# Amelie-Schreiber/ShapeMol

Hardware: AMD Instinct MI355X
Metric: molecules/sec (1000-step DDPM sample, batch 256) (higher is better)
Workload: dtype f32 (matrix operands split exactly into 3 x bf16 pieces = 24 bits, six piece products, fp32 accumulate); 1 GPU; BASELINE configs[1]: batch 256 MOSES-prior molecules (9-27 atoms) per GPU, 1000-step chain, fp32 results, k=8, synthetic shapes + hash-filled weights; besides the 5 warm-up steps an untimed 200-step chain runs first to reach the loaded clocks; batch_per_gpu=256, atoms_per_gpu=5541, total_atoms=5541, noise=device Philox, trajectories=kept in HBM, launch=hipGraph replay, parallelism=dp1 (whole batches per rank), ranks_seen=1

## Files before the change

shapemol_amd/csrc/shapemol_hip.hip:

```cpp
#include "../../include/shapemol_hip.h"
#include "sm_device.h"
#include "sm_edge.h"
#include "sm_edge_bf16.h"
#include "sm_edge16.h"
#include "sm_node.h"
#include "sm_node16.h"
#include "sm_edge_stream.h"
#include "sm_misc.h"
#include "sm_cfg.h"
#include "sm_guide_groups.h"
#include "sm_mesh.h"
#include <hip/hip_ext.h>

#include <algorithm>
#include <cmath>
#include <cstdio>
#include <cstring>
#include <map>
#include <string>
#include <type_traits>
#include <vector>

#include "sm_pack.h"
#include "sm_devmem.h"
// ... 349 lines not shown
int launch_mlp2(shapemol_ctx *c, hipStream_t s, const char *name, const DevMlpImg &m, const float *in0, const float *in1,
                int mode, const float *resid, float *out, int ld_out, int n_store, int n_atoms) {
    NodeMlpArgs a{};
    a.in0 = in0; a.in1 = in1; a.w1img = c->P(m.w1img); a.b1 = c->P(m.b1); a.ln_g = c->P(m.g); a.ln_b = c->P(m.be);
    a.w2img = c->P(m.w2img); a.b2 = c->P(m.b2); a.resid = resid; a.out = out; a.ld_out = ld_out; a.n_store = n_store;
    a.mode = mode; a.nt2 = m.nt2; a.n_atoms = n_atoms;
    const int n_ct = (n_atoms + 15) / 16, teams = NodeMlpLds<H>::TEAMS;
    LAUNCH(name, SMK((node_mlp2_kernel<H, KT>), dim3((n_ct + teams - 1) / teams), dim3(kNodeThreads), 0, s, a));
    return 0;
}

template <int H>
int launch_linear(shapemol_ctx *c, hipStream_t s, const char *name, const float *in, const float *wimg, const float *wimg6, const float *wimg16, const float *add_mol,
                  int ld_add, float *out, int ld_out, int n_out_tiles, int n_atoms, unsigned long long *stamps) {
    const lg::LinGeom g = lg::linear_geom(launch_in<H>(c, n_atoms), n_out_tiles);
    const dim3 grid(g.ogroups * g.agroups), block(g.waves * 64);
    const bool f16 = c->opt.lin_bf16 && c->opt.node_f16;
    NodeLinArgs a{in, f16 ? wimg16 : (c->opt.lin_bf16 ? wimg6 : wimg), add_mol, c->mol_of, out, n_atoms, n_out_tiles, g.tpg, ld_add, ld_out, stamps, g.waves};
    if (f16) {
        const size_t shm = (size_t)std::min(g.tpg, kLin16Chunk) * 2 * H * 32;
        if (c->opt.feat_f16) LAUNCH(name, SMK((node_linear16_kernel<H, true>), grid, block, shm, s, a, c->status + ST_RANGE));
        else LAUNCH(name, SMK(node_linear16_kernel<H>, grid, block, shm, s, a, c->status + ST_RANGE));
    } else if (c->opt.lin_bf16) {
        const size_t shm = (size_t)std::min(g.tpg, kLin6Chunk) * 3 * H * 32;
        LAUNCH(name, SMK(node_linear6_kernel<H>, grid, block, shm, s, a));
    } else {
        LAUNCH(name, SMK(node_linear_kernel<H>, grid, block, 0, s, a));
    }
    return 0;
}

template <int H>
int launch_node_levels(shapemol_ctx *c, hipStream_t s, const NodeChainArgs &na, const float *lin_img6, const float *add_mol, int ld_add,
                       float *out, int ld_out, int lin_tiles, bool out_done) {
    const int n = na.n_atoms;
    const lg::NodeLevelsGeom g = lg::node_levels_geom(launch_in<H>(c, n), na.n_follow, lin_tiles);
    if (!out_done) LAUNCH("node_chain", SMK(node_out6_kernel<H>, dim3(g.n_pairs), dim3(H * 4), Out6Lds<H>::BYTES, s, na));
    NodeAfterArgs a{};
    a.f[0] = na.f[0]; a.f[1] = na.f[1];
    a.n_pairs = g.n_pairs; a.n_fjobs = g.n_fjobs; a.n_ljobs = g.n_ljobs; a.order = c->opt.after_order; a.lin_chunk = g.lin_chunk;
    a.lin = NodeLinArgs{na.h_out, lin_img6, add_mol, c->mol_of, out, n, lin_tiles, g.tpg, ld_add, ld_out, nullptr, g.lw};
    const size_t shm = After6Lds<H>::bytes(a.lin_chunk);
    const int64_t rec[8] = {1, a.n_fjobs, a.n_ljobs, g.bw, a.order, g.tpg, a.lin_chunk, (int64_t)shm};
    std::copy(rec, rec + 8, c->node_rec);
    LAUNCH("node_pre", SMK(node_after6_kernel<H>, dim3(a.n_fjobs + a.n_ljobs), dim3(g.bw * 64), shm, s, a));
    return 0;
}

NodeFollow follow_of(const shapemol_ctx *c, const DevMlpImg &m, int mode, float *out, int ld_out, int n_store) {
    NodeFollow f{};
    f.w1img = c->P(m.w1img); f.b1 = c->P(m.b1); f.ln_g = c->P(m.g); f.ln_b = c->P(m.be);
    f.w1img6 = c->P(c->opt.node_f16 ? m.w1img16 : m.w1img6); f.w2img6 = c->P(c->opt.node_f16 ? m.w2img16 : m.w2img6);
    f.w2img = c->P(m.w2img); f.b2 = c->P(m.b2); f.out = out; f.ld_out = ld_out; f.n_store = n_store; f.mode = mode; f.nt2 = m.nt2;
    return f;
}

__global__ void knn_pin_kernel(const int *off, int n_steps, const int *atom, const int *pnbr, int k, int kp, const int *step_cur, int n_atoms, int *nbr) {
    const int step = *step_cur;
    if (step < 0 || step >= n_steps) return;
    const int lo = off[step], hi = off[step + 1];
    for (int e = lo + blockIdx.x * blockDim.x + threadIdx.x; e < hi; e += gridDim.x * blockDim.x) {
        const int i = atom[e];
        if (i < 0 || i >= n_atoms) continue;
        for (int sl = 0; sl < kp; ++sl) nbr[(size_t)i * kp + sl] = sl < k ? pnbr[(size_t)e * k + sl] : -1;
    }
}

template <int H>
int run_prep_shape(shapemol_ctx *c, hipStream_t s, int64_t B, const float *d_shape, const ShapePrep &sp);

int cfg_group_blocks(int64_t n, int n_groups) { return (int)(n / 2048 + n_groups); }

CfgArgs cfg_args(const shapemol_ctx *c, int64_t N) {
    CfgArgs a{};
// ... 230 lines not shown
                sa.vf = pending;
                if (sf.out_fused) sa.no = NodeOutArgs{c->att, cur_h, c->P(Dl.no.b1), c->P(Dl.no.g), c->P(Dl.no.be), c->P(Dl.no.b2),
                                                   c->P(Dl.no.w1img6), c->P(Dl.no.w2img6), h_dst};
                if (launch_stream<H, false>(c, s, sa)) return 1;
            }
            pending = VnFold{};
            if (sf.half_tiles && launch_combine32<false>(c, s, c->att, n)) return 1;
        } else if (sf.phases && c->opt.edge_bf16 == 1) {
            EdgeFusedArgs fa{c->P(Dl.img_kx), c->P(Dl.img_vx), pre_x, c->q_x, cur_x, c->nbr, c->ew, c->alpha, c->att, n, ld_pre_x, stamps_x};
            if (launch_fused<H, false>(c, s, fa)) return 1;
        } else {
            EdgeArgs e{c->P(Dl.blob_x2h), pre_x, c->q_x, cur_x, c->nbr, c->ew, c->att, n, ld_pre_x, stamps_x};
            if (launch_edge<H, false>(c, s, e)) return 1;
        }
        {
            float *dst = h_dst;
            NodeChainArgs na{};
            na.att = c->att; na.h = cur_h; na.h_out = dst; na.n_atoms = n;
            na.stamps = (c->kstamp_sel == 3 && l == 0) ? c->kstamps : nullptr;
            na.w1img = c->P(Dl.no.w1img); na.b1 = c->P(Dl.no.b1); na.ln_g = c->P(Dl.no.g); na.ln_b = c->P(Dl.no.be);
            na.w2img = c->P(Dl.no.w2img); na.b2 = c->P(Dl.no.b2);
            na.w1img6 = c->P(c->opt.node_f16 ? Dl.no.w1img16 : Dl.no.w1img6); na.w2img6 = c->P(c->opt.node_f16 ? Dl.no.w2img16 : Dl.no.w2img6);
            na.f[0] = follow_of(c, Dl.q_h2x, NODE_LN_RELU, c->q_h, H, H);
            na.n_follow = 1;
            if (has_next) { na.f[1] = follow_of(c, c->dm.layer[l + 1].q_x2h, NODE_LN_RELU, c->q_x, H, H); na.n_follow = 2; }
            else if (out_v) { na.f[1] = follow_of(c, c->dm.vhead, NODE_SSP, out_v, C, C); na.n_follow = 2; v_done = true; }
            const int n_ct = (n + 15) / 16;
            const int lin_tiles = (has_next && l + 1 < L ? 8 : 4) * NT;
            if (sf.lin_fused) {
                na.lin_img16 = c->P(Dl.lin16_img); na.add_mol = sp.addp + (size_t)l * c->capB * 8 * H; na.mol_of = c->mol_of;
                na.pre_out = c->preAB; na.n_lin_tiles = lin_tiles; na.ld_add = 8 * H; na.ld_out = 8 * H;
            }
            float *lin_add = sp.addp + (size_t)l * c->capB * 8 * H;
            if (sf.levels) { if (launch_node_levels<H>(c, s, na, c->P(Dl.lin6_img), lin_add, 8 * H, c->preAB, 8 * H, lin_tiles, sf.out_fused)) return 1; }
            else if (sf.xc_fused) { rec[4] = 1; if (launch_x2h_chain<H>(c, s, xea, na)) return 1; }
            else if (c->opt.chain_bf16 && c->opt.node_f16 && c->opt.feat_f16) LAUNCH("node_chain", SMK((node_chain16_kernel<H, true>), dim3((n_ct + CHAIN_COLS - 1) / CHAIN_COLS), dim3(H * 4), Chain16Lds<H>::BYTES, s, na, c->status + ST_RANGE));
            else if (c->opt.chain_bf16 && c->opt.node_f16) LAUNCH("node_chain", SMK(node_chain16_kernel<H>, dim3((n_ct + CHAIN_COLS - 1) / CHAIN_COLS), dim3(H * 4), Chain16Lds<H>::BYTES, s, na, c->status + ST_RANGE));
            else if (c->opt.chain_bf16) LAUNCH("node_chain", SMK(node_chain6_kernel<H>, dim3((n_ct + CHAIN_COLS - 1) / CHAIN_COLS), dim3(H * 4), Chain6Lds<H>::BYTES, s, na));
            else LAUNCH("node_chain", SMK(node_chain_kernel<H>, dim3((n_ct + CHAIN_COLS - 1) / CHAIN_COLS), dim3(H * 4), 0, s, na));
            cur_h = dst;
            if (!sf.lin_fused && !sf.levels && launch_linear<H>(c, s, "node_pre", cur_h, c->P(Dl.lin_img), c->P(Dl.lin6_img), c->P(Dl.lin16_img), lin_add, 8 * H,
                                 c->preAB, 8 * H, lin_tiles, n, (c->kstamp_sel == 0 && l == 0) ? c->kstamps : nullptr)) return 1;
        }
        float *x_next = (last && out_pos) ? out_pos : ((cur_x == c->x_a) ? c->x_b : c->x_a);
        bool vn_done = false, stats_done = false;
        unsigned long long *stamps_h = (c->kstamp_sel == 2 && l == 0) ? c->kstamps : nullptr;
        if ((sf.f16 || sf.stream) && c->opt.vn_fuse != 1) {
            const H2xPlan plan = h2x_plan(c, sp, l, sf.fold, has_next, sf.half_tiles, stat_acc, cur_x, x_next, out_pos);
            pending = plan.pending; stats_done = plan.stats_done; vn_done = plan.vn_done;
            if (plan.ddpm.enable) c->ddpm_vf = plan.ddpm;
            rec[2] |= plan.pending.enable; rec[3] |= plan.ddpm.enable;
            if (sf.f16) {
                Edge16Args ea{};
                ea.image_k = c->P(Dl.i16_kh); ea.image_v = c->P(Dl.i16_vh);
                fill_edge(ea, c, c->preAB, 8 * H, c->q_h, cur_x, c->o3, n, sf.half_tiles, stamps_h);
                ea.vn = plan.vn; ea.xsum = plan.xsum;
                if (launch_edge16<H, true>(c, s, ea)) return 1;
            } else {
                EdgeStreamArgs sa{};
                sa.part_k = c->P(Dl.st_kh); sa.part_v = c->P(Dl.st_vh);
                sa.w2k = reinterpret_cast<const unsigned *>(c->P(Dl.sw2_kh));
                fill_edge(sa, c, c->preAB, 8 * H, c->q_h, cur_x, c->o3, n, sf.half_tiles, stamps_h);
                sa.vn = plan.vn; sa.xsum = plan.xsum;
                if (launch_stream<H, true>(c, s, sa)) return 1;
            }
            if (sf.half_tiles && launch_combine32<true>(c, s, c->o3, n)) return 1;
        } else if (sf.phases) {
// ... 290 lines not shown
    if (k == "first_step") {
        if (value < 0 || value >= c->cfg.num_timesteps) return fail("first_step must be in [0, num_timesteps)");
        c->first_step = (int)value;
        return 0;
    }
    if (k == "stop_layer") c->opt.stop_layer = (int)value;
    else if (k == "edge_bf16") {
        if (value < 0 || value > 3) return fail("edge_bf16 must be 0 (fp32 MFMA), 1 (exactly split bf16, phase kernels), 2 (exactly split bf16, streaming kernels) or 3 (two-piece f16)");
        if (value != 3 && value != 2 && c->KP > 16) return fail("k > 16 runs on the streaming (edge_bf16 = 2) or the two-piece f16 (edge_bf16 = 3) edge kernels");
        if (value == 3 && c->hid_max > 6.0e4f) return fail("edge_bf16 = 3: the edge MLPs' LayerNorm outputs may exceed the fp16 range for these weights");
        c->opt.edge_bf16 = (int)value;
    }
    else if (k == "edge_tiles") { if (value < -1 || value > 1) return fail("edge_tiles must be -1 (automatic), 0 (sliced one-job launches) or 1 (looping launch)"); c->opt.edge_tiles = (int)value; }
    else if (k == "node_f16") c->opt.node_f16 = value != 0;
    else if (k == "feat_f16") {
        if (value && (c->opt.edge_bf16 != 3 || !c->opt.node_f16)) return fail("feat_f16 = 1 needs the f16 kernels (edge_bf16 = 3, node_f16 = 1)");
        c->opt.feat_f16 = value != 0;
    }
    else if (k == "lin_fuse") c->opt.lin_fuse = value != 0;
    else if (k == "stream_whole_rounds") c->opt.stream_whole_rounds = value != 0;
    else if (k == "x2h_chain") c->opt.x2h_chain = value != 0;
    else if (k == "graph_fuse") c->opt.graph_fuse = value != 0;
    else if (k == "bn_eval") c->bn_eval = value != 0;
    else if (k == "ddpm_fold") c->opt.ddpm_fold = value != 0;
    else if (k == "vn_fold") c->opt.vn_fold = value != 0;
    else if (k == "prologue_tab") c->opt.prologue_tab = value != 0;
    else if (k == "lin_bf16") c->opt.lin_bf16 = (int)value;
    else if (k == "chain_bf16") c->opt.chain_bf16 = (int)value;
    else if (k == "vn_fuse") c->opt.vn_fuse = (int)value;
    else if (k == "node_levels") c->opt.node_levels = value != 0;
    else if (k == "x2h_out_fuse") { if (value < 0 || value > 2) return fail("x2h_out_fuse must be 0 (node_out6_kernel), 1 (x2h tail inside its boundary) or 2 (x2h tail always)"); c->opt.x2h_out_fuse = (int)value; }
    else if (k == "stream_chunk") { if (value < 0 || value > 4096) return fail("stream_chunk must be 0 (automatic) .. 4096"); c->opt.stream_chunk_opt = (int)value; }
    else if (k == "after_order") { if (value < 0 || value > 2) return fail("after_order must be 0 (follow-up jobs first), 1 (interleaved) or 2 (linear jobs first)"); c->opt.after_order = (int)value; }
    else if (k == "after_waves") { if (value < 1 || value > 16) return fail("after_waves must be 1..16"); c->opt.after_waves = (int)value; }
    else if (k == "after_lin_wgs") { if (value < 0 || value > 4096) return fail("after_lin_wgs must be 0 (automatic) .. 4096"); c->opt.after_lin_wgs = (int)value; }
    else if (k == "lin_waves") { if (value < 1 || value > 16) return fail("lin_waves must be 1..16"); c->opt.lin_waves = (int)value; }
    else if (k == "stamps") c->stamp_on = (int)value;
    else if (k == "kstamp_sel") c->kstamp_sel = (int)value;
    else if (k == "edge_waves") { if (value < 0 || value > 12) return fail("edge_waves must be 0 (automatic) .. 12"); c->opt.edge_threads = (int)value * 64; }
    else return fail("unknown option " + k);
    hipSetDevice(c->device);
    c->drop_graphs();
    return 0;
}

int64_t shapemol_debug_read(shapemol_ctx *c, const char *name, void *dst, size_t max_bytes) {
    if (!c || !name || !dst) { fail("shapemol_debug_read: null argument"); return -1; }
    const std::string k(name);
    const shapemol_config &g = c->cfg;
    const int64_t N = c->lastN;
    const void *src = nullptr; size_t bytes = 0;
    int64_t dims[8] = {N, c->lastB, c->KP, g.hidden_dim, g.n_heads, g.num_layers, c->capN, c->capB};
    if (k == "dims") { if (max_bytes < sizeof(dims)) return -1; std::memcpy(dst, dims, sizeof(dims)); return sizeof(dims); }
    if (k == "captures") { if (max_bytes < 8) return -1; std::memcpy(dst, &c->n_captures, 8); return 8; }
    if (k == "launch") { if (max_bytes < sizeof(c->launch_rec)) return -1; std::memcpy(dst, c->launch_rec, sizeof(c->launch_rec)); return sizeof(c->launch_rec); }
    if (k == "launch_x2h_out") { if (max_bytes < sizeof(c->x2h_out_rec)) return -1; std::memcpy(dst, c->x2h_out_rec, sizeof(c->x2h_out_rec)); return sizeof(c->x2h_out_rec); }
    if (k == "launch_node") { if (max_bytes < sizeof(c->node_rec)) return -1; std::memcpy(dst, c->node_rec, sizeof(c->node_rec)); return sizeof(c->node_rec); }
    if (k == "nbr") { src = c->nbr; bytes = N * c->KP * 4; }
    else if (k == "ew") { src = c->ew; bytes = N * c->KP * 4; }
    else if (k == "h") { src = c->last_h; bytes = N * g.hidden_dim * 4; }
    else if (k == "x") { src = c->last_x; bytes = N * 3 * 4; }
    else if (k == "h0") { src = c->h_a; bytes = N * g.hidden_dim * 4; }
    else if (k == "q_x") { src = c->q_x; bytes = N * g.hidden_dim * 4; }
    else if (k == "pre0") { src = c->pre0; bytes = N * 4 * g.hidden_dim * 4; }
    else if (k == "add0") { src = c->prep[0].add0; bytes = (size_t)c->lastB * 4 * g.hidden_dim * 4; }
    else if (k == "pre") { src = c->preAB; bytes = N * 8 * g.hidden_dim * 4; }
// ... 176 lines not shown
```

shapemol_amd/csrc/sm_device.h:

```cpp
#pragma once
#include <hip/hip_runtime.h>
#include <stdint.h>

typedef float f32x4 __attribute__((ext_vector_type(4)));

#define SM_DEV __device__ __forceinline__

#ifdef SM_STAMPS
#define SM_STAMP(buf, slot)                                                                        \
    do {                                                                                           \
        if ((buf) != nullptr && (threadIdx.x & 63) == 0) {                                         \
            unsigned long long t_;                                                                 \
            __builtin_amdgcn_sched_barrier(0);                                                     \
            asm volatile("s_waitcnt vmcnt(0) lgkmcnt(0)\n\ts_memrealtime %0\n\ts_waitcnt lgkmcnt(0)" : "=s"(t_)::"memory"); \
            __builtin_amdgcn_sched_barrier(0);                                                     \
            (buf)[(((size_t)blockIdx.y * gridDim.x + blockIdx.x) * (blockDim.x >> 6) + (threadIdx.x >> 6)) * 8 + (slot)] = t_; \
        }                                                                                          \
    } while (0)
#define SM_TICK(buf, slot)                                                                         \
    do {                                                                                           \
        if ((buf) != nullptr && (threadIdx.x & 63) == 0) {                                         \
            unsigned long long t_;                                                                 \
            __builtin_amdgcn_sched_barrier(0);                                                     \
            asm volatile("s_memrealtime %0\n\ts_waitcnt lgkmcnt(0)" : "=s"(t_)::"memory");         \
            __builtin_amdgcn_sched_barrier(0);                                                     \
            (buf)[(((size_t)blockIdx.y * gridDim.x + blockIdx.x) * (blockDim.x >> 6) + (threadIdx.x >> 6)) * 8 + (slot)] = t_; \
        }                                                                                          \
    } while (0)
#else
#define SM_STAMP(buf, slot) do { } while (0)
#define SM_TICK(buf, slot) do { } while (0)
#endif

SM_DEV f32x4 mfma16(float a, float b, f32x4 c) {
    return __builtin_amdgcn_mfma_f32_16x16x4f32(a, b, c, 0, 0, 0);
}

SM_DEV float4 ldg4(const float *p) { return *reinterpret_cast<const float4 *>(p); }
SM_DEV void stg4(float *p, float4 v) { *reinterpret_cast<float4 *>(p) = v; }

SM_DEV void copy_to_lds(float *lds, const float *g, int n4, int tid, int nthr) {
    const float4 *src = reinterpret_cast<const float4 *>(g);
    float4 *dst = reinterpret_cast<float4 *>(lds);
    constexpr int U = 8;
    int i = tid;
    for (; i + (U - 1) * nthr < n4; i += U * nthr) {
        float4 v[U];
#pragma unroll
        for (int u = 0; u < U; ++u) v[u] = src[i + u * nthr];
#pragma unroll
        for (int u = 0; u < U; ++u) dst[i + u * nthr] = v[u];
    }
    for (; i < n4; i += nthr) dst[i] = src[i];
}

SM_DEV void dma_to_lds(float *lds, const float *g, int n4, int wave, int nwave, int lane) {
    typedef __attribute__((address_space(3))) void lds_void;
    typedef __attribute__((address_space(1))) const void gbl_void;
    const int wu = __builtin_amdgcn_readfirstlane(wave);
    for (int c = wu; c < n4 / 64; c += nwave)
        __builtin_amdgcn_global_load_lds((gbl_void *)(g + ((size_t)c * 64 + lane) * 4), (lds_void *)(lds + (size_t)c * 256), 16, 0, 0);
}

SM_DEV void image_to_lds(float *lds, const float *g, int n4, int tid, int wave, int nwave, int lane) {
// ... 254 lines not shown
```

shapemol_amd/csrc/sm_launch.h:

```cpp
#pragma once
#include <algorithm>

namespace lg {

struct Options {
    int stop_layer = -1, edge_threads = 0 , lin_waves = 16, edge_bf16 = 2, lin_bf16 = 1, chain_bf16 = 1, vn_fuse = 2;
    int vn_fold = 1;
    int max_mol_atoms = 0;
    int stream_whole_rounds = 0;
    int lin_fuse = 0;
    int ddpm_fold = 1;
    int graph_fuse = 1;
    int x2h_chain = 1;
    int node_levels = 1;
    int x2h_out_fuse = 1;
    int stream_chunk_opt = 0;
    int after_order = 2;
    int after_waves = 16;
    int after_lin_wgs = 0;
    int node_f16 = 0;
    int feat_f16 = 0;
    int edge_tiles = -1;
    int prologue_tab = 1;
};

struct KernelConsts { int vn_fold_cap, stream_tpr, chain_cols, graph_cap, lin6_chunk; bool chain16_fits; };

struct In { Options o; KernelConsts k; int KP, num_cu, H, n_atoms; };

inline int cdiv(int a, int b) { return (a + b - 1) / b; }

struct Jobs { int apj, jobs; bool half; };
inline Jobs tile_jobs(int KP, int n_atoms) {
    const int apj = KP >= 16 ? 1 : 16 / KP;
    return {apj, KP > 16 ? 2 * n_atoms : cdiv(n_atoms, apj), KP > 16};
}

enum class Form { One, Loop, Sliced, Strided };
struct EdgeGeom { Form form; int apj, jobs, waves, grid, chunk, slice, atoms_per_wg; };

inline int edge_waves(const In &in, int jobs) {
    return in.o.edge_threads > 0 ? in.o.edge_threads / 64 : std::max(4, std::min(12, cdiv(jobs, in.num_cu)));
}
inline EdgeGeom one_job_geom(const In &in, int waves) {
    const Jobs j = tile_jobs(in.KP, in.n_atoms);
    const int grid = std::max(1, std::min(in.num_cu, cdiv(j.jobs, waves)));
    return {j.jobs <= grid * waves ? Form::One : Form::Strided, j.apj, j.jobs, waves, grid, waves, grid * waves, j.half ? 0 : waves * j.apj};
}

inline EdgeGeom edge_fp32_geom(const In &in) {
    const Jobs j = tile_jobs(in.KP, in.n_atoms);
    const int grid = std::max(1, std::min(in.num_cu, j.jobs));
    return {Form::Strided, j.apj, j.jobs, in.o.edge_threads > 0 ? in.o.edge_threads / 64 : 12, grid, 1, grid, 0};
}

inline EdgeGeom edge_phase_geom(const In &in) {
// ... 110 lines not shown
```

shapemol_amd/csrc/sm_node.h:

```cpp
#pragma once
#include "sm_device.h"

enum NodeMode { NODE_LN_RELU = 1, NODE_SSP = 2 };
constexpr int kNodeThreads = 1024;

struct NodeLinArgs {
    const float *in;
    const float *wimg;
    const float *add_mol;
    const int *mol_of;
    float *out;
    int n_atoms, n_out_tiles, tiles_per_group;
    int ld_add, ld_out;
    unsigned long long *stamps;
    int nwave;
};

constexpr int kLinChunk = 8;

template <int H>
__global__ void __launch_bounds__(kNodeThreads)
node_linear_kernel(NodeLinArgs a) {
    constexpr int NT = H / 16;
    constexpr int XS = H + 16;
    __shared__ __attribute__((aligned(16))) float tiles[kLinChunk * 16 * XS];
    const int lane = threadIdx.x & 63, wave = threadIdx.x >> 6;
    const int n = lane & 15, g = lane >> 4;
    const int nwave = blockDim.x >> 6;
    const int ogroups = (a.n_out_tiles + nwave - 1) / nwave;
    const int ot_raw = (blockIdx.x % ogroups) * nwave + wave;
    const bool ot_ok = ot_raw < a.n_out_tiles;
    const int ot = ot_ok ? ot_raw : a.n_out_tiles - 1;
    const int ag = blockIdx.x / ogroups;
    const int n_ct = (a.n_atoms + 15) / 16;
// ... 8 lines not shown
        const int nc = min(kLinChunk, ct1 - cb);
        __syncthreads();
        for (int idx = threadIdx.x; idx < nc * 16 * (H / 4); idx += blockDim.x) {
            const int ar = idx / (H / 4), c4 = idx % (H / 4);
            const int at = min(cb * 16 + ar, a.n_atoms - 1);
            stg4(tiles + ar * XS + 4 * c4, ldg4(a.in + (size_t)at * H + 4 * c4));
        }
        __syncthreads();
        float4 add_cur = {0.f, 0.f, 0.f, 0.f}, add_nxt = {0.f, 0.f, 0.f, 0.f};
        if (a.add_mol) add_cur = ldg4(a.add_mol + (size_t)a.mol_of[min(cb * 16 + n, a.n_atoms - 1)] * a.ld_add + 16 * ot + 4 * g);
        for (int c = 0; c < nc; ++c) {
            if (a.add_mol && c + 1 < nc)
                add_nxt = ldg4(a.add_mol + (size_t)a.mol_of[min((cb + c + 1) * 16 + n, a.n_atoms - 1)] * a.ld_add + 16 * ot + 4 * g);
            const float *xrow = tiles + (c * 16 + n) * XS;
            f32x4 acc = {add_cur.x, add_cur.y, add_cur.z, add_cur.w};
#pragma unroll
            for (int t = 0; t < NT; ++t) {
                const float4 x = ldg4(xrow + 16 * t + 4 * g);
                acc = mfma16(w[t].x, x.x, acc);
                acc = mfma16(w[t].y, x.y, acc);
                acc = mfma16(w[t].z, x.z, acc);
                acc = mfma16(w[t].w, x.w, acc);
            }
            const int atom = (cb + c) * 16 + n;
            if (ot_ok && atom < a.n_atoms) stg4(a.out + (size_t)atom * a.ld_out + 16 * ot + 4 * g, float4{acc[0], acc[1], acc[2], acc[3]});
            add_cur = add_nxt;
        }
    }
    SM_STAMP(a.stamps, 2);
}

constexpr int kLin6Chunk = 8;

template <int H>
SM_DEV void linear6_job(const NodeLinArgs &a, int job, int chunk, u32x4 *frag) {
    constexpr int NB = H / 32;
    const int lane = threadIdx.x & 63, wave = threadIdx.x >> 6;
    const int n = lane & 15, g = lane >> 4;
    const int nwave = a.nwave;
    const int ogroups = (a.n_out_tiles + nwave - 1) / nwave;
    const int ot_raw = (job % ogroups) * nwave + wave;
    const bool ot_ok = ot_raw < a.n_out_tiles;
    const int ot = ot_ok ? ot_raw : a.n_out_tiles - 1;
    const int ag = job / ogroups;
    const int n_ct = (a.n_atoms + 15) / 16;
    const int ct0 = ag * a.tiles_per_group, ct1 = min(ct0 + a.tiles_per_group, n_ct);

    u32x4 w[3][NB];
    {
        const u32x4 *wi = reinterpret_cast<const u32x4 *>(a.wimg) + (size_t)ot * 3 * NB * 64 + lane;
#pragma unroll
        for (int p = 0; p < 3; ++p)
#pragma unroll
            for (int b = 0; b < NB; ++b) w[p][b] = wi[(p * NB + b) * 64];
    }

    for (int cb = ct0; cb < ct1; cb += chunk) {
        const int nc = min(chunk, ct1 - cb);
        __syncthreads();
        for (int idx = threadIdx.x; idx < nc * NB * 64; idx += nwave * 64) {
            const int sl = idx & 63, sb = (idx >> 6) % NB, sc = idx / (64 * NB);
            const int at = min((cb + sc) * 16 + (sl & 15), a.n_atoms - 1);
            const float *src = a.in + (size_t)at * H + 32 * sb + 4 * (sl >> 4);
            const float4 v0 = ldg4(src), v1 = ldg4(src + 16);
            const float v[8] = {v0.x, v0.y, v0.z, v0.w, v1.x, v1.y, v1.z, v1.w};
            u32x4 hi, mid, lo;
            split3_bf16(v, hi, mid, lo);
            u32x4 *dst = frag + ((size_t)(sc * 3) * NB + sb) * 64 + sl;
            dst[0] = hi; dst[NB * 64] = mid; dst[2 * NB * 64] = lo;
        }
        __syncthreads();
        for (int c = 0; c < nc; c += 2) {
            const bool two = c + 1 < nc;
            const int atom0 = (cb + c) * 16 + n, atom1 = atom0 + 16;
            f32x4 acc0 = {0.f, 0.f, 0.f, 0.f}, acc1 = {0.f, 0.f, 0.f, 0.f};
            if (a.add_mol) {
                const float4 t0 = ldg4(a.add_mol + (size_t)a.mol_of[min(atom0, a.n_atoms - 1)] * a.ld_add + 16 * ot + 4 * g);
                const float4 t1 = ldg4(a.add_mol + (size_t)a.mol_of[min(atom1, a.n_atoms - 1)] * a.ld_add + 16 * ot + 4 * g);
                acc0 = f32x4{t0.x, t0.y, t0.z, t0.w}; acc1 = f32x4{t1.x, t1.y, t1.z, t1.w};
            }
            const u32x4 *f0 = frag + (size_t)(c * 3) * NB * 64 + lane;
            const u32x4 *f1 = frag + (size_t)((two ? c + 1 : c) * 3) * NB * 64 + lane;
#pragma unroll
            for (int b = 0; b < NB; ++b) {
                const u32x4 h0 = f0[b * 64], m0 = f0[(NB + b) * 64], l0 = f0[(2 * NB + b) * 64];
                const u32x4 h1 = f1[b * 64], m1 = f1[(NB + b) * 64], l1 = f1[(2 * NB + b) * 64];
                acc0 = mfma_bf16(w[2][b], h0, acc0); acc1 = mfma_bf16(w[2][b], h1, acc1);
                acc0 = mfma_bf16(w[1][b], m0, acc0); acc1 = mfma_bf16(w[1][b], m1, acc1);
                acc0 = mfma_bf16(w[0][b], l0, acc0); acc1 = mfma_bf16(w[0][b], l1, acc1);
                acc0 = mfma_bf16(w[1][b], h0, acc0); acc1 = mfma_bf16(w[1][b], h1, acc1);
                acc0 = mfma_bf16(w[0][b], m0, acc0); acc1 = mfma_bf16(w[0][b], m1, acc1);
                acc0 = mfma_bf16(w[0][b], h0, acc0); acc1 = mfma_bf16(w[0][b], h1, acc1);
            }
            if (ot_ok && atom0 < a.n_atoms) stg4(a.out + (size_t)atom0 * a.ld_out + 16 * ot + 4 * g, float4{acc0[0], acc0[1], acc0[2], acc0[3]});
            if (ot_ok && two && atom1 < a.n_atoms) stg4(a.out + (size_t)atom1 * a.ld_out + 16 * ot + 4 * g, float4{acc1[0], acc1[1], acc1[2], acc1[3]});
        }
    }
}

template <int H>
__global__ void __launch_bounds__(kNodeThreads)
node_linear6_kernel(NodeLinArgs a) {
    extern __shared__ __attribute__((aligned(16))) unsigned char lin6_lds[];
    linear6_job<H>(a, blockIdx.x, kLin6Chunk, reinterpret_cast<u32x4 *>(lin6_lds));
}

struct NodeMlpArgs {
    const float *in0;
    const float *in1;
    const float *w1img;
    const float *b1;
    const float *ln_g, *ln_b;
    const float *w2img;
    const float *b2;
    const float *resid;
    float *out;
    int ld_out, n_store, mode, nt2, n_atoms;
};

template <int H>
struct NodeMlpLds {
    static constexpr int NT = H / 16;
    static constexpr int TEAMS = (16 / NT) < 4 ? (16 / NT) : 4;
    static constexpr int XS = H + 16;
    static constexpr int TOTAL = TEAMS * 16 * XS;
};

template <int H, int KT>
__global__ void __launch_bounds__(kNodeThreads)
node_mlp2_kernel(NodeMlpArgs a) {
// ... 712 lines not shown
    SM_DEV void put_frag(u32x4 *fo, int sb, int sc, int sl, const float (&v)[8]) const {
        u32x4 hi, mid, lo;
        split3_bf16(v, hi, mid, lo);
        u32x4 *dst = fo + (sb * CC + sc) * 64 + frag_slot(sb, sl);
        dst[0] = hi; dst[KB * CC * 64] = mid; dst[2 * KB * CC * 64] = lo;
    }
    SM_DEV void normalise(const float *pre, int mode, const float *gam, const float *bet, u32x4 *fo) const {
        const int col = ot * (64 / LPC) + lane / LPC, ln = lane % LPC;
        const int b = ln >> 2, gg = ln & 3;
        const int fa = 32 * b + 4 * gg;
        const float4 p0 = ldg4(pre + col * XS + fa), p1 = ldg4(pre + col * XS + fa + 16);
        float v[8] = {p0.x, p0.y, p0.z, p0.w, p1.x, p1.y, p1.z, p1.w};
        if (mode == NODE_LN_RELU) {
            float s = 0.f;
#pragma unroll
            for (int i = 0; i < 8; ++i) s += v[i];
            const float mean = seg_sum<LPC>(s) * (1.0f / H);
            float q = 0.f;
#pragma unroll
            for (int i = 0; i < 8; ++i) { const float d = v[i] - mean; q += d * d; }
            const float var = seg_sum<LPC>(q) * (1.0f / H);
            const float rstd = 1.0f / sqrtf(var + 1e-5f);
            const float4 g0 = ldg4(gam + fa), g1 = ldg4(gam + fa + 16), b0 = ldg4(bet + fa), b1 = ldg4(bet + fa + 16);
            const float ga[8] = {g0.x, g0.y, g0.z, g0.w, g1.x, g1.y, g1.z, g1.w};
            const float be[8] = {b0.x, b0.y, b0.z, b0.w, b1.x, b1.y, b1.z, b1.w};
#pragma unroll
            for (int i = 0; i < 8; ++i) v[i] = fmaxf((v[i] - mean) * rstd * ga[i] + be[i], 0.f);
        } else {
#pragma unroll
            for (int i = 0; i < 8; ++i) v[i] = (v[i] > 20.f ? v[i] : log1pf(expf(v[i]))) - 0.6931471805599453f;
        }
        put_frag<NB>(fo, b, col >> 4, gg * 16 + (col & 15), v);
    }
};

template <int H>
struct Out6Lds {
    static constexpr size_t BYTES = (size_t)2 * Chain6Lds<H>::FRAG * 16 + (size_t)Chain6Lds<H>::PRE * 4;
};

struct NodeOutArgs {
    const float *att, *h;
    const float *b1, *ln_g, *ln_b, *b2, *w1img6, *w2img6;
    float *h_out;
};

template <int H, bool AHEAD>
SM_DEV void node_out6_pair(const NodeOutArgs &a, int atom0, int atom_end, unsigned char *lds) {
    using L = Chain6Lds<H>;
    constexpr int NT = H / 16, NB = H / 32, CC = CHAIN_COLS;
    u32x4 *fin = reinterpret_cast<u32x4 *>(lds);
    float *pre0 = reinterpret_cast<float *>(fin + 2 * L::FRAG);
    const Team6<H> t;
    auto atom_of = [&](int c) { return min(atom0 + c * 16 + t.n, atom_end - 1); };
    auto atom_ok = [&](int c) { return atom0 + c * 16 + t.n < atom_end; };

    u32x4 w1[3][2 * NB], w2[3][NB];
    constexpr int SITER = CC * 2 * NB * 64 / (NT * 64);
    float4 sv0[SITER], sv1[SITER];
#pragma unroll
    for (int it = 0; it < SITER; ++it) {
        const int idx = threadIdx.x + it * NT * 64;
        const int sl = idx & 63, sb = (idx >> 6) % (2 * NB), sc = idx / (64 * 2 * NB);
        const int at = min(atom0 + sc * 16 + (sl & 15), atom_end - 1);
        const float *src = (sb < NB ? a.att + (size_t)at * H + 32 * sb : a.h + (size_t)at * H + 32 * (sb - NB)) + 4 * (sl >> 4);
        sv0[it] = ldg4(src); sv1[it] = ldg4(src + 16);
// ... 28 lines not shown
#pragma unroll
        for (int c = 0; c < CC; ++c) hres[c] = ldg4(a.h + (size_t)atom_of(c) * H + t.f0);
        b2 = ldg4(a.b2 + t.f0);
    }
    __syncthreads();
    t.normalise(pre0, NODE_LN_RELU, a.ln_g, a.ln_b, fin);
    __syncthreads();
    f32x4 acc[CC];
#pragma unroll
    for (int c = 0; c < CC; ++c) acc[c] = f32x4{b2.x, b2.y, b2.z, b2.w};
    t.gemm6(w2, fin, acc);
#pragma unroll
    for (int c = 0; c < CC; ++c) {
        const float4 hn = {acc[c][0] + hres[c].x, acc[c][1] + hres[c].y, acc[c][2] + hres[c].z, acc[c][3] + hres[c].w};
        if (atom_ok(c)) stg4(a.h_out + (size_t)atom_of(c) * H + t.f0, hn);
    }
}

template <int H>
__global__ void __launch_bounds__(H * 4)
node_out6_kernel(NodeChainArgs a) {
    extern __shared__ __attribute__((aligned(16))) unsigned char out6_lds[];
    const NodeOutArgs o{a.att, a.h, a.b1, a.ln_g, a.ln_b, a.b2, a.w1img6, a.w2img6, a.h_out};
    node_out6_pair<H, true>(o, blockIdx.x * CHAIN_COLS * 16, a.n_atoms, out6_lds);
}

struct NodeAfterArgs {
    NodeLinArgs lin;
    NodeFollow f[2];
    int n_pairs;
    int n_fjobs, n_ljobs;
    int order;
    int lin_chunk;
};

template <int H>
struct After6Lds {
    static constexpr size_t FOLLOW = (size_t)Chain6Lds<H>::FRAG * 16 + (size_t)Chain6Lds<H>::PRE * 4;
    static constexpr size_t bytes(int lin_chunk) { const size_t l = (size_t)lin_chunk * 3 * H * 32; return l > FOLLOW ? l : FOLLOW; }
};

template <int H>
__global__ void __launch_bounds__(kNodeThreads)
node_after6_kernel(NodeAfterArgs a) {
    using L = Chain6Lds<H>;
    constexpr int NT = H / 16, NB = H / 32, CC = CHAIN_COLS;
    extern __shared__ __attribute__((aligned(16))) unsigned char after6_lds[];
    const int blk = blockIdx.x;
    int fj = -1, lj = -1;
    if (a.order == 0) { if (blk < a.n_fjobs) fj = blk; else lj = blk - a.n_fjobs; }
    else if (a.order == 2) { if (blk < a.n_ljobs) lj = blk; else fj = blk - a.n_ljobs; }
    else {
        const long long tot = a.n_fjobs + a.n_ljobs;
        const int lo = (int)((long long)blk * a.n_ljobs / tot), hi = (int)((long long)(blk + 1) * a.n_ljobs / tot);
        if (hi > lo) lj = lo; else fj = blk - lo;
    }
    if (lj >= 0) {
        if ((int)(threadIdx.x >> 6) >= a.lin.nwave) return;
        linear6_job<H>(a.lin, lj, a.lin_chunk, reinterpret_cast<u32x4 *>(after6_lds));
        return;
    }
    const Team6<H> t;
    if (t.ot >= NT) return;
    const NodeFollow &F = a.f[fj / a.n_pairs];
    const int ct0 = (fj % a.n_pairs) * CC, n_atoms = a.lin.n_atoms;
    u32x4 *fh = reinterpret_cast<u32x4 *>(after6_lds);
    float *pre = reinterpret_cast<float *>(fh + L::FRAG);

    static_assert(CC * NB * 64 == NT * 64, "one fragment per thread");
    const int sl = t.lane, sb = t.ot % NB, sc = t.ot / NB;
    const int at = min((ct0 + sc) * 16 + (sl & 15), n_atoms - 1);
    const float *src = a.lin.in + (size_t)at * H + 32 * sb + 4 * (sl >> 4);
    const float4 v0 = ldg4(src), v1 = ldg4(src + 16);
    const float4 b1 = ldg4(F.b1 + t.f0);
    u32x4 w1[3][NB], w2[3][NB];
    t.load_w(F.w1img6, w1);
    {
        const float v[8] = {v0.x, v0.y, v0.z, v0.w, v1.x, v1.y, v1.z, v1.w};
        t.template put_frag<NB>(fh, sb, sc, sl, v);
    }
    const bool on = t.ot < F.nt2;
    if (on) { t.load_piece(F.w2img6, 2, w2); t.load_piece(F.w2img6, 1, w2); }
    __syncthreads();
    {
        f32x4 acc[CC];
#pragma unroll
        for (int c = 0; c < CC; ++c) acc[c] = f32x4{b1.x, b1.y, b1.z, b1.w};
        t.gemm6(w1, fh, acc);
        t.store_pre(pre, acc);
    }
    if (on) t.load_piece(F.w2img6, 0, w2);
    __syncthreads();
    t.normalise(pre, F.mode, F.ln_g, F.ln_b, fh);
    __syncthreads();
    if (!on) return;
    const float4 b = ldg4(F.b2 + t.f0);
    f32x4 acc[CC];
#pragma unroll
    for (int c = 0; c < CC; ++c) acc[c] = f32x4{b.x, b.y, b.z, b.w};
    t.gemm6(w2, fh, acc);
#pragma unroll
    for (int c = 0; c < CC; ++c) {
        const int atom = (ct0 + c) * 16 + t.n;
        if (atom >= n_atoms) continue;
        if (t.f0 + 4 <= F.n_store && (F.ld_out & 3) == 0) {
            stg4(F.out + (size_t)atom * F.ld_out + t.f0, float4{acc[c][0], acc[c][1], acc[c][2], acc[c][3]});
        } else {
#pragma unroll
            for (int r = 0; r < 4; ++r)
                if (t.f0 + r < F.n_store) F.out[(size_t)atom * F.ld_out + t.f0 + r] = acc[c][r];
        }
    }
}
```

Baseline: 397.6 molecules/s.

## Software-pipeline loads in node_after6 linear and follow-up jobs

Adds a pipelined variant of the linear6 job in node_after6_kernel, enabled by default. It prefetches the next chunk's input rows into registers before the MFMA loop, loads the per-molecule add rows and mol_of indices one pair ahead, and marks pointers restrict. The follow-up jobs now load the LayerNorm gamma/beta and the second bias before the barrier rather than after it. The goal is to hide global-load latency behind compute, at the cost of more registers, which may lower occupancy. It also adds optional timestamp probes (kstamp_sel 6).

```diff
diff --git a/shapemol_amd/csrc/shapemol_hip.hip b/shapemol_amd/csrc/shapemol_hip.hip
--- a/shapemol_amd/csrc/shapemol_hip.hip
+++ b/shapemol_amd/csrc/shapemol_hip.hip
@@ -405,14 +405,14 @@
 
 template <int H>
 int launch_node_levels(shapemol_ctx *c, hipStream_t s, const NodeChainArgs &na, const float *lin_img6, const float *add_mol, int ld_add,
-                       float *out, int ld_out, int lin_tiles, bool out_done) {
+                       float *out, int ld_out, int lin_tiles, bool out_done, unsigned long long *stamps) {
     const int n = na.n_atoms;
     const lg::NodeLevelsGeom g = lg::node_levels_geom(launch_in<H>(c, n), na.n_follow, lin_tiles);
     if (!out_done) LAUNCH("node_chain", SMK(node_out6_kernel<H>, dim3(g.n_pairs), dim3(H * 4), Out6Lds<H>::BYTES, s, na));
     NodeAfterArgs a{};
     a.f[0] = na.f[0]; a.f[1] = na.f[1];
-    a.n_pairs = g.n_pairs; a.n_fjobs = g.n_fjobs; a.n_ljobs = g.n_ljobs; a.order = c->opt.after_order; a.lin_chunk = g.lin_chunk;
-    a.lin = NodeLinArgs{na.h_out, lin_img6, add_mol, c->mol_of, out, n, lin_tiles, g.tpg, ld_add, ld_out, nullptr, g.lw};
+    a.n_pairs = g.n_pairs; a.n_fjobs = g.n_fjobs; a.n_ljobs = g.n_ljobs; a.order = c->opt.after_order; a.lin_chunk = g.lin_chunk; a.pipe = c->opt.after_pipe;
+    a.lin = NodeLinArgs{na.h_out, lin_img6, add_mol, c->mol_of, out, n, lin_tiles, g.tpg, ld_add, ld_out, stamps, g.lw};
     const size_t shm = After6Lds<H>::bytes(a.lin_chunk);
     const int64_t rec[8] = {1, a.n_fjobs, a.n_ljobs, g.bw, a.order, g.tpg, a.lin_chunk, (int64_t)shm};
     std::copy(rec, rec + 8, c->node_rec);
@@ -709,7 +709,8 @@
                 na.pre_out = c->preAB; na.n_lin_tiles = lin_tiles; na.ld_add = 8 * H; na.ld_out = 8 * H;
             }
             float *lin_add = sp.addp + (size_t)l * c->capB * 8 * H;
-            if (sf.levels) { if (launch_node_levels<H>(c, s, na, c->P(Dl.lin6_img), lin_add, 8 * H, c->preAB, 8 * H, lin_tiles, sf.out_fused)) return 1; }
+            if (sf.levels) { if (launch_node_levels<H>(c, s, na, c->P(Dl.lin6_img), lin_add, 8 * H, c->preAB, 8 * H, lin_tiles, sf.out_fused,
+                                                          (c->kstamp_sel == 6 && l == 0) ? c->kstamps : nullptr)) return 1; }
             else if (sf.xc_fused) { rec[4] = 1; if (launch_x2h_chain<H>(c, s, xea, na)) return 1; }
             else if (c->opt.chain_bf16 && c->opt.node_f16 && c->opt.feat_f16) LAUNCH("node_chain", SMK((node_chain16_kernel<H, true>), dim3((n_ct + CHAIN_COLS - 1) / CHAIN_COLS), dim3(H * 4), Chain16Lds<H>::BYTES, s, na, c->status + ST_RANGE));
             else if (c->opt.chain_bf16 && c->opt.node_f16) LAUNCH("node_chain", SMK(node_chain16_kernel<H>, dim3((n_ct + CHAIN_COLS - 1) / CHAIN_COLS), dim3(H * 4), Chain16Lds<H>::BYTES, s, na, c->status + ST_RANGE));
@@ -1066,6 +1067,7 @@
     else if (k == "x2h_out_fuse") { if (value < 0 || value > 2) return fail("x2h_out_fuse must be 0 (node_out6_kernel), 1 (x2h tail inside its boundary) or 2 (x2h tail always)"); c->opt.x2h_out_fuse = (int)value; }
     else if (k == "stream_chunk") { if (value < 0 || value > 4096) return fail("stream_chunk must be 0 (automatic) .. 4096"); c->opt.stream_chunk_opt = (int)value; }
     else if (k == "after_order") { if (value < 0 || value > 2) return fail("after_order must be 0 (follow-up jobs first), 1 (interleaved) or 2 (linear jobs first)"); c->opt.after_order = (int)value; }
+    else if (k == "after_pipe") c->opt.after_pipe = value != 0;
     else if (k == "after_waves") { if (value < 1 || value > 16) return fail("after_waves must be 1..16"); c->opt.after_waves = (int)value; }
     else if (k == "after_lin_wgs") { if (value < 0 || value > 4096) return fail("after_lin_wgs must be 0 (automatic) .. 4096"); c->opt.after_lin_wgs = (int)value; }
     else if (k == "lin_waves") { if (value < 1 || value > 16) return fail("lin_waves must be 1..16"); c->opt.lin_waves = (int)value; }
diff --git a/shapemol_amd/csrc/sm_device.h b/shapemol_amd/csrc/sm_device.h
--- a/shapemol_amd/csrc/sm_device.h
+++ b/shapemol_amd/csrc/sm_device.h
@@ -17,19 +17,23 @@
             (buf)[(((size_t)blockIdx.y * gridDim.x + blockIdx.x) * (blockDim.x >> 6) + (threadIdx.x >> 6)) * 8 + (slot)] = t_; \
         }                                                                                          \
     } while (0)
-#define SM_TICK(buf, slot)                                                                         \
+#define SM_TICK_W(buf, width, slot)                                                                \
     do {                                                                                           \
         if ((buf) != nullptr && (threadIdx.x & 63) == 0) {                                         \
             unsigned long long t_;                                                                 \
             __builtin_amdgcn_sched_barrier(0);                                                     \
             asm volatile("s_memrealtime %0\n\ts_waitcnt lgkmcnt(0)" : "=s"(t_)::"memory");         \
             __builtin_amdgcn_sched_barrier(0);                                                     \
-            (buf)[(((size_t)blockIdx.y * gridDim.x + blockIdx.x) * (blockDim.x >> 6) + (threadIdx.x >> 6)) * 8 + (slot)] = t_; \
+            (buf)[(((size_t)blockIdx.y * gridDim.x + blockIdx.x) * (blockDim.x >> 6) + (threadIdx.x >> 6)) * (width) + (slot)] = t_; \
         }                                                                                          \
     } while (0)
+#define SM_TICK(buf, slot) SM_TICK_W(buf, 8, slot)
+#define SM_ARRIVED(v) asm volatile("" ::"v"(v))
 #else
 #define SM_STAMP(buf, slot) do { } while (0)
 #define SM_TICK(buf, slot) do { } while (0)
+#define SM_TICK_W(buf, width, slot) do { } while (0)
+#define SM_ARRIVED(v) do { } while (0)
 #endif
 
 SM_DEV f32x4 mfma16(float a, float b, f32x4 c) {
diff --git a/shapemol_amd/csrc/sm_launch.h b/shapemol_amd/csrc/sm_launch.h
--- a/shapemol_amd/csrc/sm_launch.h
+++ b/shapemol_amd/csrc/sm_launch.h
@@ -22,6 +22,7 @@
     int feat_f16 = 0;
     int edge_tiles = -1;
     int prologue_tab = 1;
+    int after_pipe = 1;
 };
 
 struct KernelConsts { int vn_fold_cap, stream_tpr, chain_cols, graph_cap, lin6_chunk; bool chain16_fits; };
diff --git a/shapemol_amd/csrc/sm_node.h b/shapemol_amd/csrc/sm_node.h
--- a/shapemol_amd/csrc/sm_node.h
+++ b/shapemol_amd/csrc/sm_node.h
@@ -1,5 +1,6 @@
 #pragma once
 #include "sm_device.h"
+#include <type_traits>
 
 enum NodeMode { NODE_LN_RELU = 1, NODE_SSP = 2 };
 constexpr int kNodeThreads = 1024;
@@ -74,8 +75,14 @@
 
 constexpr int kLin6Chunk = 8;
 
-template <int H>
-SM_DEV void linear6_job(const NodeLinArgs &a, int job, int chunk, u32x4 *frag) {
+constexpr int kLin6Ahead = 2;
+constexpr int kAfterSlots = 32;
+
+template <int H, bool PIPE>
+SM_DEV void linear6_body(const NodeLinArgs &a, std::conditional_t<PIPE, const float *__restrict__, const float *> in,
+                         std::conditional_t<PIPE, const float *__restrict__, const float *> add_mol,
+                         std::conditional_t<PIPE, const int *__restrict__, const int *> mol_of,
+                         std::conditional_t<PIPE, float *__restrict__, float *> out, int job, int chunk, u32x4 *frag) {
     constexpr int NB = H / 32;
     const int lane = threadIdx.x & 63, wave = threadIdx.x >> 6;
     const int n = lane & 15, g = lane >> 4;
@@ -87,40 +94,114 @@
     const int ag = job / ogroups;
     const int n_ct = (a.n_atoms + 15) / 16;
     const int ct0 = ag * a.tiles_per_group, ct1 = min(ct0 + a.tiles_per_group, n_ct);
-
-    u32x4 w[3][NB];
-    {
-        const u32x4 *wi = reinterpret_cast<const u32x4 *>(a.wimg) + (size_t)ot * 3 * NB * 64 + lane;
-#pragma unroll
-        for (int p = 0; p < 3; ++p)
-#pragma unroll
-            for (int b = 0; b < NB; ++b) w[p][b] = wi[(p * NB + b) * 64];
-    }
-
-    for (int cb = ct0; cb < ct1; cb += chunk) {
-        const int nc = min(chunk, ct1 - cb);
-        __syncthreads();
-        for (int idx = threadIdx.x; idx < nc * NB * 64; idx += nwave * 64) {
+    SM_TICK_W(a.stamps, kAfterSlots, 0);
+
+    auto mol_at = [&](int tile) { return mol_of[min(tile * 16 + n, a.n_atoms - 1)]; };
+    auto add_at = [&](int mol) { return ldg4(add_mol + (size_t)mol * a.ld_add + 16 * ot + 4 * g); };
+    auto advance = [&](int &cb_, int &c_) {
+        if (c_ + 2 < min(chunk, ct1 - cb_)) c_ += 2; else { cb_ += chunk; c_ = 0; }
+    };
+    auto rows_request = [&](int cb_, float4 (&s0)[kLin6Ahead], float4 (&s1)[kLin6Ahead]) {
+        const int lim = min(chunk, ct1 - cb_) * NB * 64;
+        int tid = threadIdx.x;
+        asm volatile("" : "+v"(tid));
+#pragma unroll
+        for (int it = 0; it < kLin6Ahead; ++it) {
+            const int idx = tid + it * nwave * 64;
+            if (idx >= lim) continue;
             const int sl = idx & 63, sb = (idx >> 6) % NB, sc = idx / (64 * NB);
-            const int at = min((cb + sc) * 16 + (sl & 15), a.n_atoms - 1);
-            const float *src = a.in + (size_t)at * H + 32 * sb + 4 * (sl >> 4);
-            const float4 v0 = ldg4(src), v1 = ldg4(src + 16);
-            const float v[8] = {v0.x, v0.y, v0.z, v0.w, v1.x, v1.y, v1.z, v1.w};
+            const int at = min((cb_ + sc) * 16 + (sl & 15), a.n_atoms - 1);
+            const float *src = in + (size_t)at * H + 32 * sb + 4 * (sl >> 4);
+            s0[it] = ldg4(src); s1[it] = ldg4(src + 16);
+        }
+    };
+    auto rows_put = [&](int cb_, const float4 (&s0)[kLin6Ahead], const float4 (&s1)[kLin6Ahead]) {
+        const int lim = min(chunk, ct1 - cb_) * NB * 64;
+#pragma unroll
+        for (int it = 0; it < kLin6Ahead; ++it) {
+            const int idx = threadIdx.x + it * nwave * 64;
+            if (idx >= lim) continue;
+            const int sl = idx & 63, sb = (idx >> 6) % NB, sc = idx / (64 * NB);
+            const float v[8] = {s0[it].x, s0[it].y, s0[it].z, s0[it].w, s1[it].x, s1[it].y, s1[it].z, s1[it].w};
             u32x4 hi, mid, lo;
             split3_bf16(v, hi, mid, lo);
             u32x4 *dst = frag + ((size_t)(sc * 3) * NB + sb) * 64 + sl;
             dst[0] = hi; dst[NB * 64] = mid; dst[2 * NB * 64] = lo;
         }
+    };
+
+    [[maybe_unused]] int ma0 = 0, ma1 = 0, cb1 = ct0, c1 = 0, cb2 = ct0, c2 = 0;
+    [[maybe_unused]] float4 ta0 = {0.f, 0.f, 0.f, 0.f}, ta1 = {0.f, 0.f, 0.f, 0.f};
+    [[maybe_unused]] int first0 = 0, first1 = 0;
+    if constexpr (PIPE) {
+        advance(cb1, c1); cb2 = cb1; c2 = c1;
+        if (cb2 < ct1) advance(cb2, c2);
+        first0 = mol_at(ct0); first1 = mol_at(ct0 + 1);
+        ma0 = mol_at(cb1 + c1); ma1 = mol_at(cb1 + c1 + 1);
+    }
+
+    u32x4 w[3][NB];
+    {
+        const u32x4 *wi = reinterpret_cast<const u32x4 *>(a.wimg) + (size_t)ot * 3 * NB * 64 + lane;
+#pragma unroll
+        for (int p = 0; p < 3; ++p)
+#pragma unroll
+            for (int b = 0; b < NB; ++b) w[p][b] = wi[(p * NB + b) * 64];
+    }
+
+    const bool ahead = PIPE && chunk * NB * 64 <= kLin6Ahead * nwave * 64;
+    [[maybe_unused]] float4 s0[kLin6Ahead], s1[kLin6Ahead];
+    if constexpr (PIPE) {
+        if (ahead) rows_request(ct0, s0, s1);
+        ta0 = add_at(first0); ta1 = add_at(first1);
+    }
+
+    int pair = 0;
+    for (int cb = ct0; cb < ct1; cb += chunk) {
+        const int nc = min(chunk, ct1 - cb);
+        if (!PIPE || cb > ct0) __syncthreads();
+        if (cb > ct0) SM_TICK_W(a.stamps, kAfterSlots, 20);
+        if (ahead) {
+            if constexpr (PIPE) rows_put(cb, s0, s1);
+        } else {
+            for (int idx = threadIdx.x; idx < nc * NB * 64; idx += nwave * 64) {
+                const int sl = idx & 63, sb = (idx >> 6) % NB, sc = idx / (64 * NB);
+                const int at = min((cb + sc) * 16 + (sl & 15), a.n_atoms - 1);
+                const float *src = in + (size_t)at * H + 32 * sb + 4 * (sl >> 4);
+                const float4 v0 = ldg4(src), v1 = ldg4(src + 16);
+                const float v[8] = {v0.x, v0.y, v0.z, v0.w, v1.x, v1.y, v1.z, v1.w};
+                u32x4 hi, mid, lo;
+                split3_bf16(v, hi, mid, lo);
+                u32x4 *dst = frag + ((size_t)(sc * 3) * NB + sb) * 64 + sl;
+                dst[0] = hi; dst[NB * 64] = mid; dst[2 * NB * 64] = lo;
+            }
+        }
+        SM_TICK_W(a.stamps, kAfterSlots, cb > ct0 ? 21 : 1);
         __syncthreads();
+        SM_TICK_W(a.stamps, kAfterSlots, cb > ct0 ? 22 : 2);
+        if constexpr (PIPE) {
+            if (ahead && cb + chunk < ct1) rows_request(cb + chunk, s0, s1);
+        }
         for (int c = 0; c < nc; c += 2) {
             const bool two = c + 1 < nc;
             const int atom0 = (cb + c) * 16 + n, atom1 = atom0 + 16;
+            if (pair < 8) SM_TICK_W(a.stamps, kAfterSlots, 3 + 2 * pair);
             f32x4 acc0 = {0.f, 0.f, 0.f, 0.f}, acc1 = {0.f, 0.f, 0.f, 0.f};
-            if (a.add_mol) {
-                const float4 t0 = ldg4(a.add_mol + (size_t)a.mol_of[min(atom0, a.n_atoms - 1)] * a.ld_add + 16 * ot + 4 * g);
-                const float4 t1 = ldg4(a.add_mol + (size_t)a.mol_of[min(atom1, a.n_atoms - 1)] * a.ld_add + 16 * ot + 4 * g);
+            [[maybe_unused]] int mb0 = 0, mb1 = 0;
+            [[maybe_unused]] float4 tb0 = {0.f, 0.f, 0.f, 0.f}, tb1 = {0.f, 0.f, 0.f, 0.f};
+            if constexpr (PIPE) {
+                mb0 = mol_at(cb2 + c2); mb1 = mol_at(cb2 + c2 + 1);
+                tb0 = add_at(ma0); tb1 = add_at(ma1);
+                __builtin_amdgcn_sched_barrier(0);
+                acc0 = f32x4{ta0.x, ta0.y, ta0.z, ta0.w}; acc1 = f32x4{ta1.x, ta1.y, ta1.z, ta1.w};
+            } else if (add_mol) {
+                const float4 t0 = ldg4(add_mol + (size_t)mol_of[min(atom0, a.n_atoms - 1)] * a.ld_add + 16 * ot + 4 * g);
+                const float4 t1 = ldg4(add_mol + (size_t)mol_of[min(atom1, a.n_atoms - 1)] * a.ld_add + 16 * ot + 4 * g);
                 acc0 = f32x4{t0.x, t0.y, t0.z, t0.w}; acc1 = f32x4{t1.x, t1.y, t1.z, t1.w};
             }
+            SM_ARRIVED(acc0[0]); SM_ARRIVED(acc1[0]);
+            if (pair < 8) SM_TICK_W(a.stamps, kAfterSlots, 4 + 2 * pair);
+            ++pair;
             const u32x4 *f0 = frag + (size_t)(c * 3) * NB * 64 + lane;
             const u32x4 *f1 = frag + (size_t)((two ? c + 1 : c) * 3) * NB * 64 + lane;
 #pragma unroll
@@ -134,10 +215,23 @@
                 acc0 = mfma_bf16(w[0][b], m0, acc0); acc1 = mfma_bf16(w[0][b], m1, acc1);
                 acc0 = mfma_bf16(w[0][b], h0, acc0); acc1 = mfma_bf16(w[0][b], h1, acc1);
             }
-            if (ot_ok && atom0 < a.n_atoms) stg4(a.out + (size_t)atom0 * a.ld_out + 16 * ot + 4 * g, float4{acc0[0], acc0[1], acc0[2], acc0[3]});
-            if (ot_ok && two && atom1 < a.n_atoms) stg4(a.out + (size_t)atom1 * a.ld_out + 16 * ot + 4 * g, float4{acc1[0], acc1[1], acc1[2], acc1[3]});
-        }
-    }
+            if constexpr (PIPE) {
+                ta0 = tb0; ta1 = tb1; ma0 = mb0; ma1 = mb1;
+                cb1 = cb2; c1 = c2;
+                if (cb2 < ct1) advance(cb2, c2);
+                asm volatile("" : "+v"(ta0.x), "+v"(ta1.x), "+v"(ma0), "+v"(ma1));
+                __builtin_amdgcn_sched_barrier(0);
+            }
+            if (ot_ok && atom0 < a.n_atoms) stg4(out + (size_t)atom0 * a.ld_out + 16 * ot + 4 * g, float4{acc0[0], acc0[1], acc0[2], acc0[3]});
+            if (ot_ok && two && atom1 < a.n_atoms) stg4(out + (size_t)atom1 * a.ld_out + 16 * ot + 4 * g, float4{acc1[0], acc1[1], acc1[2], acc1[3]});
+        }
+    }
+    SM_TICK_W(a.stamps, kAfterSlots, 23);
+}
+
+template <int H, bool PIPE = false>
+SM_DEV void linear6_job(const NodeLinArgs &a, int job, int chunk, u32x4 *frag) {
+    linear6_body<H, PIPE>(a, a.in, a.add_mol, a.mol_of, a.out, job, chunk, frag);
 }
 
 template <int H>
@@ -916,6 +1010,37 @@
         }
         put_frag<NB>(fo, b, col >> 4, gg * 16 + (col & 15), v);
     }
+    struct LnRegs { float4 g0, g1, b0, b1; };
+    SM_DEV LnRegs load_ln(const float *gam, const float *bet) const {
+        const int fa = 32 * ((lane % LPC) >> 2) + 4 * (lane & 3);
+        return {ldg4(gam + fa), ldg4(gam + fa + 16), ldg4(bet + fa), ldg4(bet + fa + 16)};
+    }
+    SM_DEV void normalise(const float *pre, int mode, const LnRegs &r, u32x4 *fo) const {
+        const int col = ot * (64 / LPC) + lane / LPC, ln = lane % LPC;
+        const int b = ln >> 2, gg = ln & 3;
+        const int fa = 32 * b + 4 * gg;
+        const float4 p0 = ldg4(pre + col * XS + fa), p1 = ldg4(pre + col * XS + fa + 16);
+        float v[8] = {p0.x, p0.y, p0.z, p0.w, p1.x, p1.y, p1.z, p1.w};
+        if (mode == NODE_LN_RELU) {
+            float s = 0.f;
+#pragma unroll
+            for (int i = 0; i < 8; ++i) s += v[i];
+            const float mean = seg_sum<LPC>(s) * (1.0f / H);
+            float q = 0.f;
+#pragma unroll
+            for (int i = 0; i < 8; ++i) { const float d = v[i] - mean; q += d * d; }
+            const float var = seg_sum<LPC>(q) * (1.0f / H);
+            const float rstd = 1.0f / sqrtf(var + 1e-5f);
+            const float ga[8] = {r.g0.x, r.g0.y, r.g0.z, r.g0.w, r.g1.x, r.g1.y, r.g1.z, r.g1.w};
+            const float be[8] = {r.b0.x, r.b0.y, r.b0.z, r.b0.w, r.b1.x, r.b1.y, r.b1.z, r.b1.w};
+#pragma unroll
+            for (int i = 0; i < 8; ++i) v[i] = fmaxf((v[i] - mean) * rstd * ga[i] + be[i], 0.f);
+        } else {
+#pragma unroll
+            for (int i = 0; i < 8; ++i) v[i] = (v[i] > 20.f ? v[i] : log1pf(expf(v[i]))) - 0.6931471805599453f;
+        }
+        put_frag<NB>(fo, b, col >> 4, gg * 16 + (col & 15), v);
+    }
 };
 
 template <int H>
@@ -1010,6 +1135,7 @@
     int n_fjobs, n_ljobs;
     int order;
     int lin_chunk;
+    int pipe;
 };
 
 template <int H>
@@ -1035,7 +1161,8 @@
     }
     if (lj >= 0) {
         if ((int)(threadIdx.x >> 6) >= a.lin.nwave) return;
-        linear6_job<H>(a.lin, lj, a.lin_chunk, reinterpret_cast<u32x4 *>(after6_lds));
+        if (a.pipe && a.lin.add_mol) linear6_job<H, true>(a.lin, lj, a.lin_chunk, reinterpret_cast<u32x4 *>(after6_lds));
+        else linear6_job<H, false>(a.lin, lj, a.lin_chunk, reinterpret_cast<u32x4 *>(after6_lds));
         return;
     }
     const Team6<H> t;
@@ -1044,6 +1171,8 @@
     const int ct0 = (fj % a.n_pairs) * CC, n_atoms = a.lin.n_atoms;
     u32x4 *fh = reinterpret_cast<u32x4 *>(after6_lds);
     float *pre = reinterpret_cast<float *>(fh + L::FRAG);
+    unsigned long long *const stamps = a.lin.stamps;
+    SM_TICK_W(stamps, kAfterSlots, 24);
 
     static_assert(CC * NB * 64 == NT * 64, "one fragment per thread");
     const int sl = t.lane, sb = t.ot % NB, sc = t.ot / NB;
@@ -1057,9 +1186,13 @@
         const float v[8] = {v0.x, v0.y, v0.z, v0.w, v1.x, v1.y, v1.z, v1.w};
         t.template put_frag<NB>(fh, sb, sc, sl, v);
     }
+    SM_TICK_W(stamps, kAfterSlots, 25);
     const bool on = t.ot < F.nt2;
     if (on) { t.load_piece(F.w2img6, 2, w2); t.load_piece(F.w2img6, 1, w2); }
     __syncthreads();
+    SM_TICK_W(stamps, kAfterSlots, 26);
+    SM_ARRIVED(w1[2][NB - 1][3]);
+    SM_TICK_W(stamps, kAfterSlots, 27);
     {
         f32x4 acc[CC];
 #pragma unroll
@@ -1068,11 +1201,22 @@
         t.store_pre(pre, acc);
     }
     if (on) t.load_piece(F.w2img6, 0, w2);
-    __syncthreads();
-    t.normalise(pre, F.mode, F.ln_g, F.ln_b, fh);
-    __syncthreads();
+    float4 b = {0.f, 0.f, 0.f, 0.f};
+    typename Team6<H>::LnRegs lnr = {b, b, b, b};
+    if (a.pipe) {
+        if (on) b = ldg4(F.b2 + t.f0);
+        if (F.mode == NODE_LN_RELU) lnr = t.load_ln(F.ln_g, F.ln_b);
+    }
+    __syncthreads();
+    SM_TICK_W(stamps, kAfterSlots, 28);
+    if (a.pipe) t.normalise(pre, F.mode, lnr, fh);
+    else t.normalise(pre, F.mode, F.ln_g, F.ln_b, fh);
+    __syncthreads();
+    SM_TICK_W(stamps, kAfterSlots, 29);
     if (!on) return;
-    const float4 b = ldg4(F.b2 + t.f0);
+    if (!a.pipe) b = ldg4(F.b2 + t.f0);
+    SM_ARRIVED(b.x);
+    SM_TICK_W(stamps, kAfterSlots, 30);
     f32x4 acc[CC];
 #pragma unroll
     for (int c = 0; c < CC; ++c) acc[c] = f32x4{b.x, b.y, b.z, b.w};
@@ -1089,4 +1233,5 @@
                 if (t.f0 + r < F.n_store) F.out[(size_t)atom * F.ld_out + t.f0 + r] = acc[c][r];
         }
     }
+    SM_TICK_W(stamps, kAfterSlots, 31);
 }
```

Result: no change. 401.2 molecules/s (median of 6 runs) (+0.9%).
